# chrished/DEMC.jl

Measured on AMD Instinct MI355X. Metric: chain-updates/sec (N x gens/s) + gens-to-Rhat<1.05, MvNormal d=5 N=1024, higher is better.
Workload: dtype f64

## Files before the change

demc.jl_amd/_lib.py:

```python
from __future__ import annotations

import ctypes as C
import os
import subprocess
from pathlib import Path

import numpy as np

PKG_DIR = Path(__file__).resolve().parent
REPO_ROOT = PKG_DIR.parent
LIB_PATH = Path(os.environ["DEMCZ_LIB"]) if os.environ.get("DEMCZ_LIB") else PKG_DIR / "libdemcz_hip.so"
ABI_VERSION = 1
LAYOUT_SPLIT = 100
LAYOUT_SPLIT_WAVE = 164
LAYOUT_PROGRAM_WAVE = 264

TARGET_MVNORMAL, TARGET_ISO_QUAD, TARGET_LINREG_SSE, TARGET_HOST_CALLBACK, TARGET_PROGRAM = 0, 1, 2, 3, 4
OK, ERR_INVALID_ARGUMENT, ERR_HIP, ERR_CAPACITY, ERR_STATE, ERR_NO_DEVICE, ERR_COMM = range(7)

_dp = C.POINTER(C.c_double)
_ip = C.POINTER(C.c_int32)
_lp = C.POINTER(C.c_int64)
_up = C.POINTER(C.c_uint64)

SYMBOLS = [
    "demcz_abi_version", "demcz_create", "demcz_destroy", "demcz_last_error", "demcz_set_state",
    "demcz_get_state", "demcz_set_history_origin", "demcz_run", "demcz_synchronize",
    "demcz_get_history", "demcz_get_changed", "demcz_rhat", "demcz_accept_ratio", "demcz_mean_cov",
    "demcz_propose", "demcz_accept_commit", "demcz_end_generation", "demcz_comm_unique_id",
    "demcz_comm_init", "demcz_export_current_device", "demcz_append_rows_device",
    "demcz_set_external_append", "demcz_get_info", "demcz_selftest_draws", "demcz_append_rows",
    "demcz_rhat_partial", "demcz_set_rng_offset", "demcz_rhat_array", "demcz_accept_ratio_array",
    "demcz_mean_cov_array", "demcz_set_append_lag", "demcz_run_checked", "demcz_set_kernel_timing",
    "demcz_get_kernel_time", "demcz_set_live_spin_limit", "demcz_get_live_status",
    "demcz_debug_append_slab", "demcz_get_changed_total", "demcz_debug_set_live_fault",
    "demcz_set_comm_timeout", "demcz_debug_stall_exchange", "demcz_get_kernel_time_series",
    "demcz_history_stream", "demcz_get_history_view", "demcz_detach_history", "demcz_release_host_buffer", "demcz_get_archive_pinned",
    "demcz_debug_kernel_counts", "demcz_pool_trim", "demcz_debug_kernel_name", "demcz_peer_group", "demcz_get_peer_status", "demcz_peer_export", "demcz_peer_attach",
    "demcz_peer_detach", "demcz_get_peer_ping", "demcz_set_live_rearms", "demcz_get_live_rearms",
    "demcz_closure_buffers", "demcz_program_check", "demcz_set_program",
    "demcz_program_check_layout",
    "demcz_autocov_sums", "demcz_autocov_sums_array", "demcz_ess_from_sums", "demcz_ess", "demcz_ess_array",
    "demcz_quantile_plan", "demcz_select_counts", "demcz_select_step", "demcz_quantile_finish", "demcz_quantiles",
    "demcz_quantiles_array", "demcz_best", "demcz_best_array",
    "demcz_derive_check", "demcz_derive", "demcz_derive_array",
]


class DemczError(RuntimeError):
    def __init__(self, code: int, msg: str):
        super().__init__(f"libdemcz_hip status {code}: {msg}")
        self.code = code


class Config(C.Structure):
    _fields_ = [
        ("N", C.c_int64), ("chain_id0", C.c_int64), ("d", C.c_int32), ("K", C.c_int32),
        ("Mcap", C.c_int64), ("Gcap", C.c_int64), ("Nblocks", C.c_int32),
        ("block_offsets", _ip), ("block_indices", _ip), ("eps_scale", _dp),
        ("seed", C.c_uint64), ("device_id", C.c_int32), ("target_kind", C.c_int32),
        ("mu", _dp), ("W", _dp), ("c0", C.c_double), ("design", _dp), ("yobs", _dp),
        ("nobs", C.c_int64), ("stream", C.c_void_p), ("lanes_per_chain", C.c_int32),
        ("reserved0", C.c_int32),
    ]


HIPCC_FLAGS = ["-O3", "--offload-arch=gfx950", "-ffp-contract=off", "-fPIC", "-Werror", "-Wno-pass-failed"]


def sources() -> list:
    csrc = PKG_DIR / "csrc"
    return ([csrc / "demcz_capi.hip"] + sorted(csrc.glob("demcz_pw_inst_*.hip")) + sorted(csrc.glob("demcz_mlr_inst_*.hip"))
            + [csrc / "demcz_program.hip"])


def build_command(out: Path = LIB_PATH) -> list:
    return ["hipcc"] + HIPCC_FLAGS + ["-shared", "-o", str(out)] + [str(p) for p in sources()] + ["-lrccl", "-lhiprtc"]

# ... 89 lines not shown
    L.demcz_get_info.argtypes = [C.c_void_p, _lp, _lp, _ip]
    L.demcz_selftest_draws.argtypes = [C.c_int32, C.c_uint64, C.c_uint64, C.c_uint64, C.c_int32,
                                       C.POINTER(C.c_uint64), _dp, _dp]
    L.demcz_set_live_spin_limit.argtypes = [C.c_void_p, C.c_int32]
    L.demcz_get_live_status.argtypes = [C.c_void_p, _ip, _ip]
    L.demcz_debug_kernel_counts.argtypes = [C.c_void_p, _lp]
    L.demcz_history_stream.argtypes = [C.c_void_p, C.c_int32]
    L.demcz_get_history_view.argtypes = [C.c_void_p, C.c_int64, C.c_int64, C.POINTER(C.c_void_p), C.POINTER(C.c_void_p)]
    L.demcz_detach_history.argtypes = [C.c_void_p, C.POINTER(C.c_void_p), C.POINTER(C.c_void_p)]
    L.demcz_release_host_buffer.argtypes = [C.c_void_p]
    L.demcz_pool_trim.argtypes = [_lp, _lp]
    L.demcz_peer_group.argtypes = [C.POINTER(C.c_void_p), C.c_int32]
    L.demcz_get_peer_status.argtypes = [C.c_void_p, _ip, _ip]
    L.demcz_peer_export.argtypes = [C.c_void_p, C.c_int32, C.c_int32, C.c_void_p]
    L.demcz_peer_attach.argtypes = [C.c_void_p, C.c_void_p]
    L.demcz_peer_detach.argtypes = [C.c_void_p]
    L.demcz_get_peer_ping.argtypes = [C.c_void_p, _ip, _dp]
    L.demcz_set_live_rearms.argtypes = [C.c_void_p, C.c_int32]
    L.demcz_get_live_rearms.argtypes = [C.c_void_p, _ip, _ip]
    L.demcz_debug_kernel_name.argtypes = [C.c_void_p, C.c_char_p, C.c_int32]
    L.demcz_program_check.argtypes = [C.c_int32, C.c_char_p, C.c_char_p]
    L.demcz_program_check_layout.argtypes = [C.c_int32, C.c_char_p, C.c_char_p, C.c_int32]
    L.demcz_set_program.argtypes = [C.c_void_p, C.c_char_p, C.c_char_p, _dp, C.c_int64]
    L.demcz_derive_check.argtypes = [C.c_int32, C.c_int32, C.c_char_p, C.c_char_p]
    L.demcz_derive.argtypes = [C.c_void_p, C.c_int64, C.c_int64, C.c_int32, C.c_char_p, C.c_char_p, _dp, C.c_int64, C.POINTER(C.c_void_p)]
    L.demcz_derive_array.argtypes = [C.c_int32, _dp, _dp, C.c_int64, C.c_int32, C.c_int64, C.c_int32, C.c_char_p, C.c_char_p, _dp,
                                     C.c_int64, C.POINTER(C.c_void_p)]
    L.demcz_get_archive_pinned.argtypes =[C.c_void_p, C.POINTER(C.c_void_p), _lp]
    L.demcz_get_kernel_time_series.argtypes = [C.c_void_p, C.c_int32, _dp, _dp, _ip]
    L.demcz_set_comm_timeout.argtypes = [C.c_void_p, C.c_int64]
    L.demcz_debug_stall_exchange.argtypes = [C.c_void_p, C.c_int32]
    L.demcz_debug_set_live_fault.argtypes = [C.c_void_p, C.c_int32, C.c_int64]
    L.demcz_debug_append_slab.argtypes = [C.c_void_p, _dp, C.c_int32, C.c_int32, C.c_int32]
    for name in SYMBOLS:
        fn = getattr(L, name)
        if name != "demcz_last_error":
            fn.restype = C.c_int32
    _LIB = L
    return L


def derive_launch_constants() -> tuple:
    import re
    text = (PKG_DIR / "csrc" / "demcz_kernels_derive.h").read_text()
    return tuple(int(re.search(rf"constexpr int {name} = (\d+);", text).group(1)) for name in ("DERIVE_THREADS", "DERIVE_MAX_WG"))


def f64(a, order="C"):
    return np.require(a, dtype=np.float64, requirements=["F" if order == "F" else "C", "A"])


def ptr(a, t=_dp):
    return a.ctypes.data_as(t) if a is not None else None
```

demc.jl_amd/csrc/demcz_capi.hip:

```cpp
#include "../../include/demcz.h"
#include "demcz_kernels.h"
#include "demcz_kernels_acf.h"
#include "demcz_kernels_sel.h"
#include "demcz_select_host.h"
#include "demcz_slab_plan.h"
#include "demcz_run_plan.h"
#include "demcz_kernels_ml.h"
#include "demcz_kernels_pc.h"
#include "demcz_kernels_lr.h"
#include "demcz_kernels_ps.h"
#include "demcz_kernels_ps2.h"
#include "demcz_kernels_ps2d.h"
#include "demcz_pw_dispatch.h"
#include "demcz_mlr_dispatch.h"
#include "demcz_program.h"

#include <rccl/rccl.h>

#include <algorithm>
#include <chrono>
#include <thread>
#include <cstdlib>
#include <deque>
#include <mutex>
// ... 211 lines not shown
    double* d_spec_X = nullptr;
    double* d_spec_lp = nullptr;
    hipEvent_t spec_ev = nullptr;
    double* pinned_rhat = nullptr;
    unsigned int* pinned_err = nullptr;
    int64_t pinned_err_launches = -1;
    int64_t pinned_cap = 0;
    bool timing = false;
    std::vector<std::pair<hipEvent_t, hipEvent_t>> timed;
    std::vector<int32_t> timed_slabs;
    std::vector<double> series_start_ms, series_dur_ms;
    int64_t timed_launches = 0;
    int64_t live_wg_cap = -1;
    SplitKind split_kind = SPLIT_NONE;
    int split_lanes = 0;
    int split_per_wg = 1;
    int32_t* d_slot_role = nullptr;
    double* d_rec[2] = {nullptr, nullptr};
    unsigned int* d_live_err = nullptr;
#ifdef DEMCZ_STAMPS
    unsigned long long* d_stamps = nullptr;
#endif
    bool arena = false, rec_in_arena = false, hist_joint = false;
    int64_t arena_gens = 0;
    int64_t arena_span = 0;
    double* arena_rec[2] = {nullptr, nullptr};
    double* arena_temp = nullptr;
    int64_t rec_cap = 0;
    int rec_cur = 0;
    bool host_paced = false;
    int wpw = 1;
    bool ps_dual = false;
    bool dual_now = false;
    bool lr_spec = false;
    bool no_live = false;
    bool live_claimed = false;
    unsigned int live_spin_limit = 0;
    int32_t live_fault_polls = 0;
    int64_t live_fault_g = 0;
    bool in_checked = false;
    struct RunCall { int64_t g_from, g_to; double gamma; bool tempered; std::vector<double> temperature; };
    std::vector<RunCall> live_log;
    double* d_safe_X = nullptr;
    double* d_safe_lp = nullptr;
    bool snap_pending = false;
    int64_t safe_M = 0, safe_M_app = 0, safe_g_done = 0;
    bool replaying = false;
    int32_t live_redos = 0;
    int32_t live_rearms_left = 3;
    int32_t live_rearms = 0;
    int64_t rearm_from = -1;
    uint32_t fail_row_hint = 0xffffffffu;
    RecDesc rec_desc[2];
    hipStream_t prod_stream = nullptr;
    hipEvent_t prod_done[2] = {nullptr, nullptr};
    hipEvent_t prod_gate = nullptr;
    bool prod_pending[2] = {false, false};
    hipEvent_t after_launch_ev = nullptr;
    unsigned int* d_acc = nullptr;
    int64_t acc_waves = 0;
    int32_t acc_slots = 0, acc_next = 0;
    struct LaunchRec { int64_t g_first, g_last; int32_t slot; };
    std::deque<LaunchRec> acc_log;
    ncclComm_t comm = nullptr;
    ncclComm_t comm_side = nullptr;
    int nranks = 1, rank = 0;
// ... 408 lines not shown
    case DEMCZ_TARGET_PROGRAM:
        if (cfg->lanes_per_chain != 0 && cfg->lanes_per_chain != 1 && cfg->lanes_per_chain != DEMCZ_LAYOUT_PROGRAM_WAVE)
            return fail(nullptr, DEMCZ_ERR_INVALID_ARGUMENT, "demcz_create: a program target runs one lane per chain: lanes_per_chain must be 0 or 1 "
                                                             "(or DEMCZ_LAYOUT_PROGRAM_WAVE: one wavefront per chain)");
        if (cfg->d > demcz_prog::MAX_PROGRAM_D)
            return fail(nullptr, DEMCZ_ERR_INVALID_ARGUMENT, "demcz_create: a program target needs 1 <= d <= 32");
        if (cfg->lanes_per_chain == DEMCZ_LAYOUT_PROGRAM_WAVE) {
            bool one_block = cfg->Nblocks == 1 && cfg->block_offsets[1] == d;
            for (int p = 0; one_block && p < d; ++p) one_block = cfg->block_indices[p] == p;
            if (!one_block)
                return fail(nullptr, DEMCZ_ERR_INVALID_ARGUMENT, "demcz_create: DEMCZ_LAYOUT_PROGRAM_WAVE needs one block 0..d-1 in order (block updates run one lane per chain)");
            if (d < demcz_prog::WAVE_MIN_D)
                return fail(nullptr, DEMCZ_ERR_INVALID_ARGUMENT, "demcz_create: DEMCZ_LAYOUT_PROGRAM_WAVE needs 2 <= d <= 32");
            if (cfg->N > PS_MAX_N)
                return fail(nullptr, DEMCZ_ERR_INVALID_ARGUMENT, "demcz_create: DEMCZ_LAYOUT_PROGRAM_WAVE needs N <= " + std::to_string(PS_MAX_N) +
                                                                 " (one wavefront per chain: PS_MAX_N)");
            if (!(cfg->Mcap <= 0xffffffffll && (double)cfg->Mcap * 8.0 * (((d + 7) / 8) * 8) < 4294967296.0))
                return fail(nullptr, DEMCZ_ERR_INVALID_ARGUMENT, "demcz_create: DEMCZ_LAYOUT_PROGRAM_WAVE needs an archive reachable by 32-bit offsets: "
                                                                 "Mcap * 8 * (d rounded up to a multiple of 8) < 2^32");
        }
        break;
    default: return fail(nullptr, DEMCZ_ERR_INVALID_ARGUMENT, "unknown target_kind");
    }
    int ndev = 0;
    if (hipGetDeviceCount(&ndev) != hipSuccess || ndev < 1)
        return fail(nullptr, DEMCZ_ERR_NO_DEVICE, "demcz_create: no HIP device visible (there is no CPU fallback)");
    if (cfg->device_id < 0 || cfg->device_id >= ndev)
        return fail(nullptr, DEMCZ_ERR_INVALID_ARGUMENT, "demcz_create: device_id out of range");

    demcz_handle* h = new demcz_handle();
    h->cfg = *cfg;
    h->lanes = 1;
    if (const char* re = getenv("DEMCZ_LIVE_REARMS")) h->live_rearms_left = std::max(0, atoi(re));
    auto bail = [&](int32_t code) {
        g_create_error = h->err;
        free_all(h);
        delete h;
        return code;
    };
#define CRCHK(expr)                                                                              \
    do {                                                                                         \
        hipError_t e_ = (expr);                                                                  \
        if (e_ != hipSuccess) {                                                                  \
            h->err = std::string(#expr) + ": " + hipGetErrorString(e_);                          \
            return bail(DEMCZ_ERR_HIP);                                                          \
        }                                                                                        \
    } while (0)
    CRCHK(hipSetDevice(cfg->device_id));
    if (cfg->stream) {
        h->stream = (hipStream_t)cfg->stream;
    } else {
        CRCHK(stream_acquire(cfg->device_id, &h->stream));
        h->own_stream = true;
    }
    h->block_offsets.assign(cfg->block_offsets, cfg->block_offsets + cfg->Nblocks + 1);
    h->block_indices.assign(cfg->block_indices, cfg->block_indices + h->block_offsets.back());
    h->eps.assign(cfg->eps_scale, cfg->eps_scale + d);
    h->slot_of.assign((size_t)cfg->Nblocks * d, -1);
    h->S = 0;
    for (int ib = 0; ib < cfg->Nblocks; ++ib) {
        const int a = h->block_offsets[ib], b = h->block_offsets[ib + 1];
        for (int t = a; t < b; ++t) h->slot_of[(size_t)ib * d + h->block_indices[t]] = t - a;
        h->S += blockstep_nblk(b - a);
    }
    h->full_block = (cfg->Nblocks == 1 && h->block_offsets[1] == d);
    if (h->full_block)
// ... 563 lines not shown
static bool split_ml_available(int target_kind, int d, bool full_block, int64_t nobs)
{
    if (!full_block) return false;
    if (target_kind == DEMCZ_TARGET_MVNORMAL) return d == 20;
    return target_kind == DEMCZ_TARGET_LINREG_SSE && d == 10 && lr16_dynamic_lds<10>(nobs) <= ML_MAX_DYNAMIC_LDS;
}

static bool ps_available(int target_kind, int d)
{
    if (target_kind == DEMCZ_TARGET_MVNORMAL) return d >= 2 && d <= PW_D_MAX;
    return target_kind == DEMCZ_TARGET_ISO_QUAD && d >= PW_D_MIN && d <= PW_D_MAX;
}

static int pc_roles(int d) { return ((d == 1) ? 1 : (d + 1) / 2) + 2; }
static int64_t rec_fields(const demcz_handle* h) { return (h->split_kind == SPLIT_MLB) ? 2 * h->S : (int64_t)h->cfg.d + 2; }
static int64_t rec_roles(const demcz_handle* h) { return (h->split_kind == SPLIT_MLB) ? h->S : pc_roles(h->cfg.d); }

#ifdef DEMCZ_STAMPS
constexpr int64_t DEMCZ_STAMP_WGS = 1 << 16;
#endif

static bool pw_matrix_form(const demcz_handle* h)
{
    const char* on = getenv("DEMCZ_PW_MFMA");
    return on && atoi(on) != 0 && h->cfg.d == 20 && h->cfg.target_kind == DEMCZ_TARGET_MVNORMAL;
}

static bool pw_regular(const WindowParams& P, bool live)
{
    static const bool no_reg = getenv("DEMCZ_NO_PW_REG") != nullptr;
    return live && !no_reg && regular_passes(P.K, P.to_boundary, P.ngen, PS_R);
}

static int32_t launch_window_pc(demcz_handle* h, const WindowParams& P, const WindowKernel& k, bool live = false)
{
    const int64_t nbc = (P.N + 63) / 64;
    const bool pc_records = !(h->split_kind == SPLIT_MLB);
    const int64_t units = pc_records ? produce_units(P.N, (int)rec_roles(h), P.rec_fields, P.next_ngen) : nbc * rec_roles(h) * P.next_ngen;
    const int upw = k.waves;
    const int64_t blocks = P.consumer_blocks + (units + upw - 1) / upw;
    if (blocks <= 0) return DEMCZ_OK;
    if (h->split_kind == SPLIT_WAVE || h->lr_spec) {
        if (h->split_kind == SPLIT_WAVE && P.ZS != ((P.d <= 2) ? 2 : (P.d <= 4) ? 4 : ((P.d + 7) / 8) * 8)) return fail(h, DEMCZ_ERR_STATE, "split layout: archive row stride");
        const int bin = (P.rec_in == h->d_rec[0]) ? 0 : 1, bout = (P.rec_out == h->d_rec[0]) ? 0 : 1;
        const bool one_launch = !live && P.consumer_blocks > 0;
        if (units > 0 && one_launch && h->prod_pending[bout]) {
            HIPCHK(h, hipStreamWaitEvent(h->stream, h->prod_done[bout], 0));
            h->prod_pending[bout] = false;
        }
        if (units > 0 && !one_launch) {
            hipStream_t ps = h->stream;
            static const bool serial_env = getenv("DEMCZ_PRODUCE_SERIAL") != nullptr;
            if (P.consumer_blocks > 0 && !serial_env && h->peer_mode != 1) {
                if (!h->prod_stream) {
                    HIPCHK(h, stream_acquire(h->cfg.device_id, &h->prod_stream));
                    HIPCHK(h, hipEventCreateWithFlags(&h->prod_gate, hipEventDisableTiming));
                    for (int b = 0; b < 2; ++b) HIPCHK(h, hipEventCreateWithFlags(&h->prod_done[b], hipEventDisableTiming));
                }
                if (h->after_launch_ev) {
                    HIPCHK(h, hipStreamWaitEvent(h->prod_stream, h->after_launch_ev, 0));
                } else {
                    HIPCHK(h, hipEventRecord(h->prod_gate, h->stream));
                    HIPCHK(h, hipStreamWaitEvent(h->prod_stream, h->prod_gate, 0));
                }
                ps = h->prod_stream;
            } else if (h->prod_pending[bout]) {
                HIPCHK(h, hipStreamWaitEvent(h->stream, h->prod_done[bout], 0));
                h->prod_pending[bout] = false;
            }
            const dim3 pg((unsigned)((units + PRODUCE_WAVES - 1) / PRODUCE_WAVES)), pw(64 * PRODUCE_WAVES);
            static const size_t throttle_env = getenv("DEMCZ_PRODUCE_LDS") ? (size_t)atol(getenv("DEMCZ_PRODUCE_LDS")) : PRODUCE_THROTTLE_LDS;
            size_t big_d = throttle_env;
            if (h->split_kind == SPLIT_WAVE && P.d > 20) {
                int plds = 0;
                if (h->prog_wave && (!h->prog_ready || hipFuncGetAttribute(&plds, HIP_FUNC_ATTRIBUTE_SHARED_SIZE_BYTES, h->prog.wave[1][0]) != hipSuccess)) plds = (int)ML_MAX_DYNAMIC_LDS;
                size_t clds = (size_t)plds;
                if (!h->prog_wave) {
                    WindowKernel lk[MAX_LIVE_KERNELS];
                    const int nlk = live_kernels(h, lk);
                    for (int i = 0; i < nlk; ++i) {
                        hipFuncAttributes a{};
                        if (lk[i].fn && hipFuncGetAttributes(&a, lk[i].fn) == hipSuccess) clds = std::max(clds, (size_t)a.sharedSizeBytes);
                    }
                }
                const size_t room = (clds + 4096 < ML_MAX_DYNAMIC_LDS) ? ML_MAX_DYNAMIC_LDS - clds - 4096 : 8192;
                big_d = std::max<size_t>(8192, std::min<size_t>(throttle_env, room));
            }
            const size_t dyn = (ps != h->stream) ? (h->lr_spec ? (size_t)8192 : (h->ps_dual && !getenv("DEMCZ_PRODUCE_LDS")) ? (size_t)32768 : big_d) : 0;
            switch (P.d) {
#define DEMCZ_PRODUCE_CASE(DD) case DD: hipLaunchKernelGGL((produce_kernel<DD>), pg, pw, dyn, ps, P); break;
            DEMCZ_PRODUCE_CASE(2) DEMCZ_PRODUCE_CASE(3) DEMCZ_PRODUCE_CASE(4) DEMCZ_PRODUCE_CASE(5) DEMCZ_PRODUCE_CASE(6) DEMCZ_PRODUCE_CASE(7)
            DEMCZ_PRODUCE_CASE(8) DEMCZ_PRODUCE_CASE(9) DEMCZ_PRODUCE_CASE(10) DEMCZ_PRODUCE_CASE(11) DEMCZ_PRODUCE_CASE(12) DEMCZ_PRODUCE_CASE(13)
            DEMCZ_PRODUCE_CASE(14) DEMCZ_PRODUCE_CASE(15) DEMCZ_PRODUCE_CASE(16) DEMCZ_PRODUCE_CASE(17) DEMCZ_PRODUCE_CASE(18) DEMCZ_PRODUCE_CASE(19)
            DEMCZ_PRODUCE_CASE(20) DEMCZ_PRODUCE_CASE(21) DEMCZ_PRODUCE_CASE(22) DEMCZ_PRODUCE_CASE(23) DEMCZ_PRODUCE_CASE(24) DEMCZ_PRODUCE_CASE(25)
            DEMCZ_PRODUCE_CASE(26) DEMCZ_PRODUCE_CASE(27) DEMCZ_PRODUCE_CASE(28) DEMCZ_PRODUCE_CASE(29) DEMCZ_PRODUCE_CASE(30) DEMCZ_PRODUCE_CASE(31)
            DEMCZ_PRODUCE_CASE(32)
#undef DEMCZ_PRODUCE_CASE
            default: return fail(h, DEMCZ_ERR_STATE, "split layout: dimension not built");
            }
            HIPCHK(h, hipGetLastError());
            if (ps != h->stream) {
                HIPCHK(h, hipEventRecord(h->prod_done[bout], ps));
                h->prod_pending[bout] = true;
            }
        }
        if (P.consumer_blocks > 0) {
            if (h->prod_pending[bin]) {
                if (h->host_paced) { int32_t rcw = sync_event(h, h->prod_done[bin], "launch_window_pc"); if (rcw) return rcw; }
                else HIPCHK(h, hipStreamWaitEvent(h->stream, h->prod_done[bin], 0));
                h->prod_pending[bin] = false;
            }
            static_assert(PS_CHAINS == LR16_WAVES, "producer units per workgroup of a one-launch grid");
            const int64_t grid = P.consumer_blocks + (one_launch ? (units + PS_CHAINS - 1) / PS_CHAINS : 0);
            return launch_kernel(h, k, grid, P);
        }
        return DEMCZ_OK;
    }
    return launch_kernel(h, k, blocks, P);
}

static int32_t rec_reserve(demcz_handle* h, int64_t gens)
{
    if (gens <= h->rec_cap) return DEMCZ_OK;
    { int32_t rcq = quiesce_all(h); if (rcq) return rcq; }
    SYNCCHK(h, h->stream);
    if (h->prod_stream) SYNCCHK(h, h->prod_stream);
    h->prod_pending[0] = h->prod_pending[1] = false;
    if (h->arena && gens <= h->arena_gens && h->rec_cap == 0) {
        for (int b = 0; b < 2; ++b) { h->d_rec[b] = h->arena_rec[b]; h->rec_desc[b].valid = false; }
        h->rec_in_arena = true;
        h->rec_cap = h->arena_gens;
        return DEMCZ_OK;
    }
// ... 2957 lines not shown
    if (live_enabled) *live_enabled = (h->lanes == DEMCZ_LAYOUT_SPLIT && !h->no_live && h->live_claimed) ? 1 : 0;
    if (redos) *redos = h->live_redos;
    return DEMCZ_OK;
}

extern "C" int32_t demcz_debug_append_slab(demcz_handle* h, const double* slab, int32_t R, int32_t cnt, int32_t batched)
{
    NOT_DERIVED(h);
    if (!h || !slab || R < 1 || cnt < 1 || (!batched && cnt != 1)) return DEMCZ_ERR_INVALID_ARGUMENT;
    if (!h->has_state) return fail(h, DEMCZ_ERR_STATE, "demcz_debug_append_slab: no state");
    if (h->lag != 0 || !h->pending.empty()) return fail(h, DEMCZ_ERR_STATE, "demcz_debug_append_slab: rows are pending");
    const int64_t N = h->cfg.N, rows = N * R * cnt;
    const int d = h->cfg.d;
    if (h->M_app + rows > h->cfg.Mcap) return fail(h, DEMCZ_ERR_CAPACITY, "demcz_debug_append_slab: Z capacity exceeded");
    HIPCHK(h, hipSetDevice(h->cfg.device_id));
    int32_t rc = ensure_scratch(h, rows * d);
    if (rc) return rc;
    HIPCHK(h, hipMemcpyAsync(h->d_scratch, slab, (size_t)rows * d * sizeof(double), hipMemcpyHostToDevice, h->stream));
    const int64_t tot = rows * d;
    if (batched)
        hipLaunchKernelGGL(append_batch_kernel, dim3((unsigned)((tot + 255) / 256)), dim3(256), 0, h->stream, h->dZ, h->ZS,
                           h->M_app, (const double*)h->d_scratch, N, (int)R, (int)cnt, d);
    else
        hipLaunchKernelGGL(append_gathered_kernel, dim3((unsigned)((tot + 255) / 256)), dim3(256), 0, h->stream, h->dZ, h->ZS,
                           h->M_app, (const double*)h->d_scratch, N, (int)R, d);
    HIPCHK(h, hipGetLastError());
    SYNCCHK(h, h->stream);
    h->M_app += rows;
    h->M = h->M_app;
    rec_invalidate(h);
    return DEMCZ_OK;
}

extern "C" int32_t demcz_set_kernel_timing(demcz_handle* h, int32_t enabled)
{
    NOT_DERIVED(h);
    if (!h) return DEMCZ_ERR_INVALID_ARGUMENT;
    h->timing = enabled != 0;
    return DEMCZ_OK;
}

extern "C" int32_t demcz_get_kernel_time(demcz_handle* h, int64_t* launches, double* milliseconds)
{
    NOT_DERIVED(h);
    if (!h) return DEMCZ_ERR_INVALID_ARGUMENT;
    HIPCHK(h, hipSetDevice(h->cfg.device_id));
    SYNCCHK(h, h->stream);
    double total = 0.0;
    h->after_launch_ev = nullptr;
    h->series_start_ms.clear(); h->series_dur_ms.clear();
    for (auto& pr : h->timed) {
        float ms = 0.0f, st = 0.0f;
        HIPCHK(h, hipEventElapsedTime(&ms, pr.first, pr.second));
        if (&pr != &h->timed.front()) HIPCHK(h, hipEventElapsedTime(&st, h->timed.front().first, pr.first));
        const int32_t k = h->timed_slabs[(size_t)(&pr - &h->timed.front())];
        for (int32_t i = 0; i < k; ++i) { h->series_start_ms.push_back((double)st + i * ((double)ms / k)); h->series_dur_ms.push_back((double)ms / k); }
        total += ms;
    }
    for (auto& pr : h->timed) {
        (void)hipEventDestroy(pr.first);
        (void)hipEventDestroy(pr.second);
    }
    if (launches) *launches = h->timed_launches;
    if (milliseconds) *milliseconds = total;
    h->timed.clear();
    h->timed_slabs.clear();
// ... 17 lines not shown
```

demc.jl_amd/csrc/demcz_kernels_ps.h:

```cpp
#pragma once

#include "demcz_kernels_pc.h"

#pragma clang fp contract(off)

namespace demcz {

constexpr int PS_CHAINS = 4;
constexpr int PS_R = 5;
constexpr int PS_PUB = 4;
#ifndef PS_AHEAD_N
#define PS_AHEAD_N 2
#endif
constexpr int PS_AHEAD = PS_AHEAD_N;
constexpr int PS_SLOTS = PS_AHEAD + 1;
constexpr int PS_MAX_N = 2048;

__device__ __forceinline__ void ps_dma16(const void* gsrc, unsigned lds_dst)
{
    unsigned keep;
    asm volatile("s_mov_b32 %0, m0\n\ts_mov_b32 m0, %2\n\ts_nop 0\n\tglobal_load_lds_dwordx4 %1, off\n\ts_mov_b32 m0, %0"
                 : "=&s"(keep) : "v"(gsrc), "s"(lds_dst) : "memory");
}

constexpr int PRODUCE_WAVES = 4;
constexpr size_t PRODUCE_THROTTLE_LDS = 64 * 1024;
template <int D>
__global__ void __launch_bounds__(64 * PRODUCE_WAVES) produce_kernel(const WindowParams P)
{
    pc_produce<D>(P, (int64_t)blockIdx.x * PRODUCE_WAVES + (int64_t)(threadIdx.x >> 6), (int)(threadIdx.x & 63));
}

template <int TARGET, int D, bool LIVE, bool TEMPER>
__global__ void __launch_bounds__(64 * (PS_CHAINS + (LIVE ? 1 : 0)), 3) window_kernel_ps(const WindowParams P)
{
#ifdef DEMCZ_PROGRAM_TARGET
    static_assert(TARGET == TARGET_MVNORMAL || TARGET == TARGET_ISO_QUAD || TARGET == TARGET_PROGRAM, "split layout: MvNormal / isotropic / program targets");
#else
    static_assert(TARGET == TARGET_MVNORMAL || TARGET == TARGET_ISO_QUAD, "split layout: MvNormal / isotropic targets");
#endif
    static_assert(D >= 2 && D <= 5, "a pass's rows, normals, log u and indices are one 64-lane DMA");
    constexpr bool PROG = (TARGET == TARGET_PROGRAM);
    constexpr int HW = (D + 1) / 2;
    constexpr int ZSC = (D <= 2) ? 2 : (D <= 4) ? 4 : 8;
    constexpr int ZSH = (ZSC == 2) ? 4 : (ZSC == 4) ? 5 : 6;
    constexpr int DP = ((D + 1) / 2) * 2;
    constexpr int CR = ((D + 2) / 2) * 2;
    constexpr int ROWL = PS_R * 2 * HW;
    constexpr int FL0 = ROWL;
    constexpr int TL0 = FL0 + 3 * (D + 2);
    static_assert(TL0 + 3 <= 64, "one DMA instruction per pass");
    const int lane = threadIdx.x & 63;
    const int w = __builtin_amdgcn_readfirstlane((int)(threadIdx.x >> 6));
    if constexpr (!LIVE) {
        if ((int64_t)blockIdx.x >= P.consumer_blocks) {
            pc_produce<D>(P, ((int64_t)blockIdx.x - P.consumer_blocks) * PS_CHAINS + w, lane);
            return;
        }
    }
    __shared__ __attribute__((aligned(16))) unsigned char raw[PS_CHAINS][PS_SLOTS][1024];
    __shared__ __attribute__((aligned(16))) double sdelta[PS_CHAINS][(PS_R + 1) * DP];
    __shared__ __attribute__((aligned(16))) double ctab[PS_CHAINS][2][32 * CR];
    __shared__ double pub_rows[LIVE ? PS_CHAINS * PS_PUB * D : 1];
// ... 460 lines not shown
```

demc.jl_amd/csrc/demcz_kernels_rec.h:

```cpp
#pragma once

#include "demcz_kernels.h"

#pragma clang fp contract(off)

namespace demcz {

struct philox_blocks : rocrand_device::philox4x32_10_engine {
    __device__ __forceinline__ philox_blocks() {}
    __device__ __forceinline__ void block(uint64_t seed, uint64_t chain, uint64_t blk, uint64_t& r1, uint64_t& r2)
    {
        uint4 ctr = {(unsigned)blk, (unsigned)(blk >> 32), (unsigned)chain, (unsigned)(chain >> 32)};
        uint2 key = {(unsigned)seed, (unsigned)(seed >> 32)};
        uint4 w = this->ten_rounds(ctr, key);
        r1 = (uint64_t)w.x | ((uint64_t)w.y << 32);
        r2 = (uint64_t)w.z | ((uint64_t)w.w << 32);
    }
};

__device__ __forceinline__ void wave_lds_handoff()
{
    asm volatile("" ::: "memory");
    __builtin_amdgcn_wave_barrier();
    asm volatile("" ::: "memory");
// ... 28 lines not shown
        const int64_t plane = pb / nbc;
        c = (pb % nbc) * 64 + lane;
        role = (int)(plane % S);
        gi = (int)(plane / S);
    }
    if (gi >= P.next_ngen || c >= P.N) return;
    philox_blocks rng;
    uint64_t r1, r2;
    rng.block(P.seed, (uint64_t)(P.chain_id0 + c), (uint64_t)(P.next_g_first + gi - 1) * (uint64_t)S + (uint64_t)role, r1, r2);
    double* rec = P.rec_out;
    auto at = [&](int g, int f) -> size_t {
        return P.rec_fields ? rec_index_rm(P.N, P.rec_fields, g, f, c) : rec_index(P.N, P.rec_stride, g, f, c);
    };
    if (role == 0) {
        const int64_t Mg = P.next_M + (int64_t)((gi + P.next_boff) / P.K) * P.next_rows;
        uint64_t i1, i2;
        draw_rows(r1, r2, (uint64_t)Mg, i1, i2);
        rec[at(gi, D + 1)] = __longlong_as_double((long long)(i1 | (i2 << 32)));
    } else {
        const double lg = dm_log(u_open(r1));
        if (role == S - 1) {
            rec[at(gi, D)] = lg;
        } else {
            const double R = sqrt(-2.0 * lg);
            double cs, sn;
            dm_sincos2pi(r2 >> 11, cs, sn);
            const int p0 = (D == 1) ? 0 : 2 * (role - 1);
            rec[at(gi, p0)] = R * cs;
            if (p0 + 1 < D) rec[at(gi, p0 + 1)] = R * sn;
        }
    }
}

__device__ __forceinline__ void pcb_produce(const WindowParams& P, int64_t pb)
{
    const int64_t nbc = (P.N + 63) / 64;
    const int64_t plane = pb / nbc;
    const int64_t c = (pb % nbc) * 64 + (threadIdx.x & 63);
    const int s = (int)(plane % P.S), gi = (int)(plane / P.S);
    if (gi >= P.next_ngen || c >= P.N) return;
    const int role = P.slot_role[s];
    philox_blocks rng;
    uint64_t r1, r2;
    rng.block(P.seed, (uint64_t)(P.chain_id0 + c), (uint64_t)(P.next_g_first + gi - 1) * (uint64_t)P.S + (uint64_t)s, r1, r2);
    double2 e;
    if (role == 0) {
        const int64_t Mg = P.next_M + (int64_t)((gi + P.next_boff) / P.K) * P.next_rows;
        uint64_t i1, i2;
        draw_rows(r1, r2, (uint64_t)Mg, i1, i2);
        e.x = __longlong_as_double((long long)i1);
        e.y = __longlong_as_double((long long)i2);
    } else {
        const double lg = dm_log(u_open(r1));
        if (role == 2) {
            e.x = lg;
            e.y = 0.0;
        } else {
            const double R = sqrt(-2.0 * lg);
            double cs, sn;
            dm_sincos2pi(r2 >> 11, cs, sn);
            e.x = R * cs;
            e.y = R * sn;
        }
    }
    reinterpret_cast<double2*>(P.rec_out)[((size_t)gi * (size_t)P.N + (size_t)c) * (size_t)P.S + (size_t)s] = e;
}
// ... 59 lines not shown
```

demc.jl_amd/engine.py:

```python
from __future__ import annotations

import ctypes as C
from collections import namedtuple

import numpy as np

from . import _lib
from ._lib import DemczError
from .targets import is_device_target

ESS = namedtuple("ESS", "ess tau varplus pairs converged")


def ess_from_sums(m, n, sums, between):
    sums = _lib.f64(sums, "F")
    d, nlags = sums.shape
    between = _lib.f64(between)
    if between.shape != (d,):
        raise ValueError("between must have d entries")
    out = ESS(np.empty(d), np.empty(d), np.empty(d), np.zeros(d, dtype=np.int64), np.zeros(d, dtype=np.int32))
    rc = _lib.load().demcz_ess_from_sums(d, int(m), int(n), nlags, _lib.ptr(sums), _lib.ptr(between), _lib.ptr(out.ess), _lib.ptr(out.tau),
                                         _lib.ptr(out.varplus), _lib.ptr(out.pairs, _lib._lp), _lib.ptr(out.converged, _lib._ip))
    if rc != 0:
        raise DemczError(rc, "demcz_ess_from_sums: d >= 1, n >= 2, nlags >= 1")
# ... 490 lines not shown
        self._chk(self._L.demcz_peer_detach(self._h))

    def peer_ping(self):
        ok, us = C.c_int32(-1), C.c_double(0.0)
        self._chk(self._L.demcz_get_peer_ping(self._h, C.byref(ok), C.byref(us)))
        return int(ok.value), float(us.value)

    def peer_status(self):
        m, n = C.c_int32(0), C.c_int32(0)
        self._chk(self._L.demcz_get_peer_status(self._h, C.byref(m), C.byref(n)))
        return int(m.value), int(n.value)

    def set_comm_timeout(self, milliseconds: int):
        self._chk(self._L.demcz_set_comm_timeout(self._h, C.c_int64(int(milliseconds))))

    def debug_stall_exchange(self, milliseconds: int):
        self._chk(self._L.demcz_debug_stall_exchange(self._h, C.c_int32(int(milliseconds))))

    def set_external_append(self, enabled: bool):
        self._chk(self._L.demcz_set_external_append(self._h, 1 if enabled else 0))

    def append_rows(self, rows):
        rows = _lib.f64(rows, "F")
        if rows.ndim != 2 or rows.shape[1] != self.d:
            raise ValueError("rows must be nrows x d")
        self._chk(self._L.demcz_append_rows(self._h, _lib.ptr(rows), rows.shape[0], rows.shape[0]))

    def debug_append_slab(self, slab, R, cnt, batched):
        slab = _lib.f64(slab)
        if slab.size != R * cnt * self.d * self.N:
            raise ValueError("slab must hold R*cnt*d*N doubles")
        self._chk(self._L.demcz_debug_append_slab(self._h, _lib.ptr(slab), int(R), int(cnt), 1 if batched else 0))

    def export_current_device(self, device_ptr: int):
        self._chk(self._L.demcz_export_current_device(self._h, C.c_void_p(device_ptr)))

    def append_rows_device(self, device_ptr: int, nrows: int, ldrows: int):
        self._chk(self._L.demcz_append_rows_device(self._h, C.c_void_p(device_ptr), int(nrows), int(ldrows)))


def pool_trim():
    L = _lib.load()
    a, b = C.c_int64(0), C.c_int64(0)
    L.demcz_pool_trim(C.byref(a), C.byref(b))
    return int(a.value), int(b.value)


def selftest_draws(seed, chain, blk0, n, device_id=0):
    L = _lib.load()
    words = np.zeros(2 * n, dtype=np.uint64)
    normals = np.zeros(2 * n)
    logu = np.zeros(n)
    rc = L.demcz_selftest_draws(int(device_id), int(seed), int(chain), int(blk0), int(n),
                                words.ctypes.data_as(C.POINTER(C.c_uint64)), _lib.ptr(normals), _lib.ptr(logu))
    if rc != 0:
        raise DemczError(rc, (L.demcz_last_error(None) or b"").decode())
    return words.reshape(n, 2), normals.reshape(n, 2), logu
```

include/demcz.h:

```cpp
#ifndef DEMCZ_H
#define DEMCZ_H

#include <stdint.h>

#ifdef __cplusplus
extern "C" {
#endif

typedef struct demcz_handle demcz_handle;

enum demcz_status {
    DEMCZ_OK = 0,
    DEMCZ_ERR_INVALID_ARGUMENT = 1,
    DEMCZ_ERR_HIP = 2,
    DEMCZ_ERR_CAPACITY = 3,
    DEMCZ_ERR_STATE = 4,
    DEMCZ_ERR_NO_DEVICE = 5,
    DEMCZ_ERR_COMM = 6
};

enum demcz_target_kind {
    DEMCZ_TARGET_MVNORMAL = 0,
    DEMCZ_TARGET_ISO_QUAD = 1,
    DEMCZ_TARGET_LINREG_SSE = 2,
// ... 137 lines not shown
                     const double* data, int64_t ndata, demcz_handle** derived);
int32_t demcz_derive_array(int32_t device_id, const double* chain, const double* log_obj ,
                           int64_t N, int32_t d, int64_t G, int32_t m, const char* source, const char* options,
                           const double* data, int64_t ndata, demcz_handle** derived);

int32_t demcz_get_info(const demcz_handle* h, int64_t* M, int64_t* launches_window, int32_t* lanes_per_chain);

int32_t demcz_run_checked(demcz_handle* h, int64_t g_from, int64_t g_to, double gamma, const double* temperature,
                          int64_t every, double threshold, int64_t* g_stop, int32_t* n_checks,
                          double* rhat_max, int32_t n_max, double* rhat_last);


int32_t demcz_set_kernel_timing(demcz_handle* h, int32_t enabled);
int32_t demcz_get_kernel_time(demcz_handle* h, int64_t* launches, double* milliseconds);

int32_t demcz_get_kernel_time_series(demcz_handle* h, int32_t cap, double* start_ms, double* duration_ms, int32_t* n);

int32_t demcz_selftest_draws(int32_t device_id, uint64_t seed, uint64_t chain, uint64_t blk0, int32_t n,
                             uint64_t* words, double* normals, double* logu);

int32_t demcz_set_live_spin_limit(demcz_handle* h, int32_t polls);
int32_t demcz_get_live_status(const demcz_handle* h, int32_t* live_enabled, int32_t* redos);
int32_t demcz_set_live_rearms(demcz_handle* h, int32_t n);
int32_t demcz_get_live_rearms(const demcz_handle* h, int32_t* rearms, int32_t* left);
int32_t demcz_debug_kernel_counts(const demcz_handle* h, int64_t* counts);
int32_t demcz_debug_kernel_name(const demcz_handle* h, char* buf, int32_t cap);

int32_t demcz_debug_set_live_fault(demcz_handle* h, int32_t polls, int64_t g_from);

int32_t demcz_debug_stall_exchange(demcz_handle* h, int32_t milliseconds);

int32_t demcz_debug_append_slab(demcz_handle* h, const double* slab, int32_t R, int32_t cnt, int32_t batched);

#ifdef __cplusplus
}
#endif
#endif
```

Before: 724.4 million.

## Add generation-parallel produce kernel for random-draw record buffers

```diff
diff --git a/demc.jl_amd/_lib.py b/demc.jl_amd/_lib.py
--- a/demc.jl_amd/_lib.py
+++ b/demc.jl_amd/_lib.py
@@ -44,6 +44,7 @@
     "demcz_quantile_plan", "demcz_select_counts", "demcz_select_step", "demcz_quantile_finish", "demcz_quantiles",
     "demcz_quantiles_array", "demcz_best", "demcz_best_array",
     "demcz_derive_check", "demcz_derive", "demcz_derive_array",
+    "demcz_debug_produce",
 ]
 
 
@@ -199,6 +200,7 @@
     L.demcz_debug_stall_exchange.argtypes = [C.c_void_p, C.c_int32]
     L.demcz_debug_set_live_fault.argtypes = [C.c_void_p, C.c_int32, C.c_int64]
     L.demcz_debug_append_slab.argtypes = [C.c_void_p, _dp, C.c_int32, C.c_int32, C.c_int32]
+    L.demcz_debug_produce.argtypes = [C.c_void_p, C.c_int64, C.c_int32, C.c_int64, C.c_int64, C.c_int32, C.c_int32, _dp, _lp]
     for name in SYMBOLS:
         fn = getattr(L, name)
         if name != "demcz_last_error":
diff --git a/demc.jl_amd/csrc/demcz_capi.hip b/demc.jl_amd/csrc/demcz_capi.hip
--- a/demc.jl_amd/csrc/demcz_capi.hip
+++ b/demc.jl_amd/csrc/demcz_capi.hip
@@ -267,6 +267,7 @@
     int wpw = 1;
     bool ps_dual = false;
     bool dual_now = false;
+    bool produce_units = false;
     bool lr_spec = false;
     bool no_live = false;
     bool live_claimed = false;
@@ -741,6 +742,7 @@
     h->cfg = *cfg;
     h->lanes = 1;
     if (const char* re = getenv("DEMCZ_LIVE_REARMS")) h->live_rearms_left = std::max(0, atoi(re));
+    h->produce_units = getenv("DEMCZ_NO_PRODUCE_GEN") != nullptr;
     auto bail = [&](int32_t code) {
         g_create_error = h->err;
         free_all(h);
@@ -1370,6 +1372,45 @@
     return live && !no_reg && regular_passes(P.K, P.to_boundary, P.ngen, PS_R);
 }
 
+static int32_t launch_produce(demcz_handle* h, const WindowParams& P, int64_t units, hipStream_t ps, size_t dyn, bool by_unit)
+{
+    const int64_t gwg = ((int64_t)P.next_ngen + PRODUCE_GENS_PER_WG - 1) / PRODUCE_GENS_PER_WG;
+    if (!produce_by_generation(P.rec_fields, P.next_ngen) || P.N > 0x7fffffffll || gwg > 65535) by_unit = true;
+    if (by_unit) {
+        const dim3 pg((unsigned)((units + PRODUCE_WAVES - 1) / PRODUCE_WAVES)), pw(64 * PRODUCE_WAVES);
+        switch (P.d) {
+#define DEMCZ_PRODUCE_CASE(DD) case DD: hipLaunchKernelGGL((produce_kernel<DD>), pg, pw, dyn, ps, P); break;
+        DEMCZ_PRODUCE_CASE(2) DEMCZ_PRODUCE_CASE(3) DEMCZ_PRODUCE_CASE(4) DEMCZ_PRODUCE_CASE(5) DEMCZ_PRODUCE_CASE(6) DEMCZ_PRODUCE_CASE(7)
+        DEMCZ_PRODUCE_CASE(8) DEMCZ_PRODUCE_CASE(9) DEMCZ_PRODUCE_CASE(10) DEMCZ_PRODUCE_CASE(11) DEMCZ_PRODUCE_CASE(12) DEMCZ_PRODUCE_CASE(13)
+        DEMCZ_PRODUCE_CASE(14) DEMCZ_PRODUCE_CASE(15) DEMCZ_PRODUCE_CASE(16) DEMCZ_PRODUCE_CASE(17) DEMCZ_PRODUCE_CASE(18) DEMCZ_PRODUCE_CASE(19)
+        DEMCZ_PRODUCE_CASE(20) DEMCZ_PRODUCE_CASE(21) DEMCZ_PRODUCE_CASE(22) DEMCZ_PRODUCE_CASE(23) DEMCZ_PRODUCE_CASE(24) DEMCZ_PRODUCE_CASE(25)
+        DEMCZ_PRODUCE_CASE(26) DEMCZ_PRODUCE_CASE(27) DEMCZ_PRODUCE_CASE(28) DEMCZ_PRODUCE_CASE(29) DEMCZ_PRODUCE_CASE(30) DEMCZ_PRODUCE_CASE(31)
+        DEMCZ_PRODUCE_CASE(32)
+#undef DEMCZ_PRODUCE_CASE
+        default: return fail(h, DEMCZ_ERR_STATE, "split layout: dimension not built");
+        }
+    } else {
+        ProduceParams Q;
+        Q.seed = P.seed; Q.chain_id0 = P.chain_id0; Q.N = P.N; Q.rec_out = P.rec_out; Q.rec_stride = P.rec_stride;
+        Q.next_g_first = P.next_g_first; Q.next_M = P.next_M; Q.next_rows = P.next_rows;
+        Q.next_ngen = P.next_ngen; Q.next_boff = P.next_boff; Q.K = P.K;
+        const dim3 pg((unsigned)P.N, (unsigned)gwg), pw(64 * PRODUCE_GEN_WAVES);
+        switch (P.d) {
+#define DEMCZ_PRODUCE_CASE(DD) case DD: hipLaunchKernelGGL((produce_gen_kernel<DD>), pg, pw, dyn, ps, Q); break;
+        DEMCZ_PRODUCE_CASE(2) DEMCZ_PRODUCE_CASE(3) DEMCZ_PRODUCE_CASE(4) DEMCZ_PRODUCE_CASE(5) DEMCZ_PRODUCE_CASE(6) DEMCZ_PRODUCE_CASE(7)
+        DEMCZ_PRODUCE_CASE(8) DEMCZ_PRODUCE_CASE(9) DEMCZ_PRODUCE_CASE(10) DEMCZ_PRODUCE_CASE(11) DEMCZ_PRODUCE_CASE(12) DEMCZ_PRODUCE_CASE(13)
+        DEMCZ_PRODUCE_CASE(14) DEMCZ_PRODUCE_CASE(15) DEMCZ_PRODUCE_CASE(16) DEMCZ_PRODUCE_CASE(17) DEMCZ_PRODUCE_CASE(18) DEMCZ_PRODUCE_CASE(19)
+        DEMCZ_PRODUCE_CASE(20) DEMCZ_PRODUCE_CASE(21) DEMCZ_PRODUCE_CASE(22) DEMCZ_PRODUCE_CASE(23) DEMCZ_PRODUCE_CASE(24) DEMCZ_PRODUCE_CASE(25)
+        DEMCZ_PRODUCE_CASE(26) DEMCZ_PRODUCE_CASE(27) DEMCZ_PRODUCE_CASE(28) DEMCZ_PRODUCE_CASE(29) DEMCZ_PRODUCE_CASE(30) DEMCZ_PRODUCE_CASE(31)
+        DEMCZ_PRODUCE_CASE(32)
+#undef DEMCZ_PRODUCE_CASE
+        default: return fail(h, DEMCZ_ERR_STATE, "split layout: dimension not built");
+        }
+    }
+    HIPCHK(h, hipGetLastError());
+    return DEMCZ_OK;
+}
+
 static int32_t launch_window_pc(demcz_handle* h, const WindowParams& P, const WindowKernel& k, bool live = false)
 {
     const int64_t nbc = (P.N + 63) / 64;
@@ -1406,7 +1447,6 @@
                 HIPCHK(h, hipStreamWaitEvent(h->stream, h->prod_done[bout], 0));
                 h->prod_pending[bout] = false;
             }
-            const dim3 pg((unsigned)((units + PRODUCE_WAVES - 1) / PRODUCE_WAVES)), pw(64 * PRODUCE_WAVES);
             static const size_t throttle_env = getenv("DEMCZ_PRODUCE_LDS") ? (size_t)atol(getenv("DEMCZ_PRODUCE_LDS")) : PRODUCE_THROTTLE_LDS;
             size_t big_d = throttle_env;
             if (h->split_kind == SPLIT_WAVE && P.d > 20) {
@@ -1425,18 +1465,7 @@
                 big_d = std::max<size_t>(8192, std::min<size_t>(throttle_env, room));
             }
             const size_t dyn = (ps != h->stream) ? (h->lr_spec ? (size_t)8192 : (h->ps_dual && !getenv("DEMCZ_PRODUCE_LDS")) ? (size_t)32768 : big_d) : 0;
-            switch (P.d) {
-#define DEMCZ_PRODUCE_CASE(DD) case DD: hipLaunchKernelGGL((produce_kernel<DD>), pg, pw, dyn, ps, P); break;
-            DEMCZ_PRODUCE_CASE(2) DEMCZ_PRODUCE_CASE(3) DEMCZ_PRODUCE_CASE(4) DEMCZ_PRODUCE_CASE(5) DEMCZ_PRODUCE_CASE(6) DEMCZ_PRODUCE_CASE(7)
-            DEMCZ_PRODUCE_CASE(8) DEMCZ_PRODUCE_CASE(9) DEMCZ_PRODUCE_CASE(10) DEMCZ_PRODUCE_CASE(11) DEMCZ_PRODUCE_CASE(12) DEMCZ_PRODUCE_CASE(13)
-            DEMCZ_PRODUCE_CASE(14) DEMCZ_PRODUCE_CASE(15) DEMCZ_PRODUCE_CASE(16) DEMCZ_PRODUCE_CASE(17) DEMCZ_PRODUCE_CASE(18) DEMCZ_PRODUCE_CASE(19)
-            DEMCZ_PRODUCE_CASE(20) DEMCZ_PRODUCE_CASE(21) DEMCZ_PRODUCE_CASE(22) DEMCZ_PRODUCE_CASE(23) DEMCZ_PRODUCE_CASE(24) DEMCZ_PRODUCE_CASE(25)
-            DEMCZ_PRODUCE_CASE(26) DEMCZ_PRODUCE_CASE(27) DEMCZ_PRODUCE_CASE(28) DEMCZ_PRODUCE_CASE(29) DEMCZ_PRODUCE_CASE(30) DEMCZ_PRODUCE_CASE(31)
-            DEMCZ_PRODUCE_CASE(32)
-#undef DEMCZ_PRODUCE_CASE
-            default: return fail(h, DEMCZ_ERR_STATE, "split layout: dimension not built");
-            }
-            HIPCHK(h, hipGetLastError());
+            { int32_t rcp = launch_produce(h, P, units, ps, dyn, h->produce_units); if (rcp) return rcp; }
             if (ps != h->stream) {
                 HIPCHK(h, hipEventRecord(h->prod_done[bout], ps));
                 h->prod_pending[bout] = true;
@@ -4460,6 +4489,34 @@
     return DEMCZ_OK;
 }
 
+constexpr int DEMCZ_PRODUCE_CANARY = 0xA5;
+extern "C" int32_t demcz_debug_produce(demcz_handle* h, int64_t g_first, int32_t ngen, int64_t M, int64_t rows, int32_t boff, int32_t form,
+                                       double* out, int64_t* rec_stride)
+{
+    NOT_DERIVED(h);
+    if (!h || (!out && !rec_stride) || g_first < 1 || ngen < 1 || M < 2 || rows < 0 || boff < 0 || boff >= h->cfg.K || (form != 0 && form != 1)) return DEMCZ_ERR_INVALID_ARGUMENT;
+    if (h->lanes != DEMCZ_LAYOUT_SPLIT || h->split_kind != SPLIT_WAVE) return fail(h, DEMCZ_ERR_STATE, "demcz_debug_produce: not the wave-per-chain layout");
+    HIPCHK(h, hipSetDevice(h->cfg.device_id));
+    { int32_t rcr = rec_reserve(h, ((int64_t)(ngen + 63) / 64 + 1) * 64); if (rcr) return rcr; }
+    if (rec_stride) *rec_stride = h->rec_cap;
+    if (!out) return DEMCZ_OK;
+    rec_invalidate(h);
+    SYNCCHK(h, h->stream);
+    double* buf = h->d_rec[h->rec_cur ^ 1];
+    const size_t nd = (size_t)h->rec_cap * (size_t)(h->cfg.d + 2) * (size_t)h->cfg.N;
+    HIPCHK(h, hipMemsetAsync(buf, DEMCZ_PRODUCE_CANARY, nd * sizeof(double), h->stream));
+    WindowParams P{};
+    P.N = h->cfg.N; P.chain_id0 = h->cfg.chain_id0; P.d = h->cfg.d; P.seed = h->cfg.seed; P.K = h->cfg.K;
+    P.rec_out = buf; P.rec_stride = h->rec_cap; P.rec_fields = 0;
+    P.next_g_first = g_first; P.next_ngen = ngen; P.next_M = M; P.next_rows = rows; P.next_boff = boff;
+    const int64_t units = produce_units(P.N, (int)rec_roles(h), P.rec_fields, P.next_ngen);
+    { int32_t rcp = launch_produce(h, P, units, h->stream, 0, form == 0); if (rcp) return rcp; }
+    HIPCHK(h, hipMemcpyAsync(out, buf, nd * sizeof(double), hipMemcpyDeviceToHost, h->stream));
+    HIPCHK(h, hipMemsetAsync(buf, 0, nd * sizeof(double), h->stream));
+    SYNCCHK(h, h->stream);
+    return DEMCZ_OK;
+}
+
 extern "C" int32_t demcz_set_kernel_timing(demcz_handle* h, int32_t enabled)
 {
     NOT_DERIVED(h);
diff --git a/demc.jl_amd/csrc/demcz_kernels_ps.h b/demc.jl_amd/csrc/demcz_kernels_ps.h
--- a/demc.jl_amd/csrc/demcz_kernels_ps.h
+++ b/demc.jl_amd/csrc/demcz_kernels_ps.h
@@ -29,6 +29,30 @@
 __global__ void __launch_bounds__(64 * PRODUCE_WAVES) produce_kernel(const WindowParams P)
 {
     pc_produce<D>(P, (int64_t)blockIdx.x * PRODUCE_WAVES + (int64_t)(threadIdx.x >> 6), (int)(threadIdx.x & 63));
+}
+
+#ifndef DEMCZ_PRODUCE_GB
+#define DEMCZ_PRODUCE_GB 1
+#endif
+constexpr int PRODUCE_GB = DEMCZ_PRODUCE_GB;
+#ifndef DEMCZ_PRODUCE_GEN_WAVES
+#define DEMCZ_PRODUCE_GEN_WAVES 2
+#endif
+constexpr int PRODUCE_GEN_WAVES = DEMCZ_PRODUCE_GEN_WAVES;
+constexpr int PRODUCE_GENS_PER_WG = 64 * PRODUCE_GEN_WAVES * PRODUCE_GB;
+template <int D>
+__global__ void __launch_bounds__(64 * PRODUCE_GEN_WAVES) produce_gen_kernel(const ProduceParams Q)
+{
+    const int wv = __builtin_amdgcn_readfirstlane((int)(threadIdx.x >> 6));
+    const int lane = (int)(threadIdx.x & 63);
+    const int64_t c = (int64_t)blockIdx.x;
+    if (c >= Q.N) return;
+    int g0 = ((int)blockIdx.y * PRODUCE_GEN_WAVES + wv) * (64 * PRODUCE_GB);
+#pragma unroll 1
+    for (int b = 0; b < PRODUCE_GB; ++b, g0 += 64) {
+        if (g0 >= Q.next_ngen) return;
+        if (g0 + lane < Q.next_ngen) pg_generation<D>(Q, c, g0 + lane);
+    }
 }
 
 template <int TARGET, int D, bool LIVE, bool TEMPER>
diff --git a/demc.jl_amd/csrc/demcz_kernels_rec.h b/demc.jl_amd/csrc/demcz_kernels_rec.h
--- a/demc.jl_amd/csrc/demcz_kernels_rec.h
+++ b/demc.jl_amd/csrc/demcz_kernels_rec.h
@@ -84,6 +84,79 @@
     }
 }
 
+struct ProduceParams {
+    uint64_t seed;
+    int64_t chain_id0;
+    int64_t N;
+    double* rec_out;
+    int64_t rec_stride;
+    int64_t next_g_first;
+    int64_t next_M;
+    int64_t next_rows;
+    int32_t next_ngen;
+    int32_t next_boff;
+    int32_t K;
+};
+
+__device__ __forceinline__ void rec_store(double* p, double v)
+{
+#ifdef DEMCZ_PRODUCE_NT
+    __builtin_nontemporal_store(v, p);
+#else
+    *p = v;
+#endif
+}
+
+#ifndef DEMCZ_PRODUCE_GROUP
+#define DEMCZ_PRODUCE_GROUP 4
+#endif
+constexpr int PRODUCE_GROUP = DEMCZ_PRODUCE_GROUP;
+
+template <int D>
+__device__ __forceinline__ void pg_generation(const ProduceParams& Q, int64_t c, int gi)
+{
+    constexpr int NPAIRS = (D == 1) ? 1 : (D + 1) / 2;
+    constexpr int S = NPAIRS + 2;
+    constexpr int FULL = D / 2;
+    philox_blocks rng;
+    const uint64_t chain = (uint64_t)(Q.chain_id0 + c);
+    const uint64_t blk0 = (uint64_t)(Q.next_g_first + gi - 1) * (uint64_t)S;
+    double* rec = Q.rec_out;
+    {
+        uint64_t r1, r2;
+        rng.block(Q.seed, chain, blk0, r1, r2);
+        const int64_t Mg = Q.next_M + (int64_t)((gi + Q.next_boff) / Q.K) * Q.next_rows;
+        uint64_t i1, i2;
+        draw_rows(r1, r2, (uint64_t)Mg, i1, i2);
+        rec_store(rec + rec_index(Q.N, Q.rec_stride, gi, D + 1, c), __longlong_as_double((long long)(i1 | (i2 << 32))));
+    }
+#pragma clang loop unroll_count(PRODUCE_GROUP)
+    for (int p = 0; p < FULL; ++p) {
+        uint64_t r1, r2;
+        rng.block(Q.seed, chain, blk0 + (uint64_t)(p + 1), r1, r2);
+        const double lg = dm_log(u_open(r1));
+        const double R = sqrt(-2.0 * lg);
+        double cs, sn;
+        dm_sincos2pi(r2 >> 11, cs, sn);
+        rec_store(rec + rec_index(Q.N, Q.rec_stride, gi, 2 * p, c), R * cs);
+        rec_store(rec + rec_index(Q.N, Q.rec_stride, gi, 2 * p + 1, c), R * sn);
+    }
+    if constexpr (D & 1) {
+        uint64_t r1, r2;
+        rng.block(Q.seed, chain, blk0 + (uint64_t)NPAIRS, r1, r2);
+        const double lg = dm_log(u_open(r1));
+        const double R = sqrt(-2.0 * lg);
+        double cs, sn;
+        dm_sincos2pi(r2 >> 11, cs, sn);
+        rec_store(rec + rec_index(Q.N, Q.rec_stride, gi, D - 1, c), R * cs);
+    }
+    {
+        uint64_t r1, r2;
+        rng.block(Q.seed, chain, blk0 + (uint64_t)(S - 1), r1, r2);
+        rec_store(rec + rec_index(Q.N, Q.rec_stride, gi, D, c), dm_log(u_open(r1)));
+    }
+}
+
 __device__ __forceinline__ void pcb_produce(const WindowParams& P, int64_t pb)
 {
     const int64_t nbc = (P.N + 63) / 64;
diff --git a/demc.jl_amd/engine.py b/demc.jl_amd/engine.py
--- a/demc.jl_amd/engine.py
+++ b/demc.jl_amd/engine.py
@@ -546,6 +546,14 @@
             raise ValueError("slab must hold R*cnt*d*N doubles")
         self._chk(self._L.demcz_debug_append_slab(self._h, _lib.ptr(slab), int(R), int(cnt), 1 if batched else 0))
 
+    def debug_produce(self, g_first, ngen, M, rows, boff, form):
+        gs = C.c_int64()
+        args = (C.c_int64(int(g_first)), C.c_int32(int(ngen)), C.c_int64(int(M)), C.c_int64(int(rows)), C.c_int32(int(boff)), C.c_int32(int(form)))
+        self._chk(self._L.demcz_debug_produce(self._h, *args, None, C.byref(gs)))
+        out = np.empty((self.d + 2, self.N, gs.value))
+        self._chk(self._L.demcz_debug_produce(self._h, *args, _lib.ptr(out), C.byref(gs)))
+        return out
+
     def export_current_device(self, device_ptr: int):
         self._chk(self._L.demcz_export_current_device(self._h, C.c_void_p(device_ptr)))
 
diff --git a/include/demcz.h b/include/demcz.h
--- a/include/demcz.h
+++ b/include/demcz.h
@@ -193,6 +193,9 @@
 
 int32_t demcz_debug_append_slab(demcz_handle* h, const double* slab, int32_t R, int32_t cnt, int32_t batched);
 
+int32_t demcz_debug_produce(demcz_handle* h, int64_t g_first, int32_t ngen, int64_t M, int64_t rows, int32_t boff, int32_t form,
+                            double* out, int64_t* rec_stride);
+
 #ifdef __cplusplus
 }
 #endif
```

Measured after the change: 720.9 million. About the same (-0.5%).
